# huttered40/capital

Measured on AMD Instinct MI355X. Metric: TFLOP/s (whole node) Cholesky n=65536, algorithmic n^3/3, recursive cholinv factor(), inputs resident in HBM, higher is better.
Workload: dtype f64

## Files before the change

capital_amd/csrc/capi_internal.h:

```cpp
#pragma once
#include <hip/hip_runtime.h>
#include <stdint.h>
#include <stdio.h>
#include <string.h>
#include "capital_hip.h"

struct capi_handle_s {
  int device = 0;
  hipStream_t stream = nullptr;
  bool owns_stream = false;
  static constexpr int NSTREAMS = 4;
  hipStream_t streams[NSTREAMS] = {nullptr, nullptr, nullptr, nullptr};
  int cur = 0;
  int cu_of[NSTREAMS] = {0, 0, 0, 0};
  hipEvent_t* events = nullptr;
  void* ws[NSTREAMS] = {nullptr, nullptr, nullptr, nullptr};
  size_t ws_bytes[NSTREAMS] = {0, 0, 0, 0};
  void* ws2[NSTREAMS] = {nullptr, nullptr, nullptr, nullptr};
  size_t ws2_bytes[NSTREAMS] = {0, 0, 0, 0};
  void* ws3[NSTREAMS] = {nullptr, nullptr, nullptr, nullptr};
  size_t ws3_bytes[NSTREAMS] = {0, 0, 0, 0};
  void* ws4[NSTREAMS] = {nullptr, nullptr, nullptr, nullptr};
  size_t ws4_bytes[NSTREAMS] = {0, 0, 0, 0};
  int* d_info = nullptr;
// ... 32 lines not shown
  do {                                                                                       \
    hipError_t e__ = (call);                                                                 \
    if (e__ != hipSuccess) {                                                                 \
      if (h) snprintf((h)->err, sizeof((h)->err), "%s:%d %s -> %s", __FILE__, __LINE__, #call, hipGetErrorString(e__)); \
      return CAPI_EHIP;                                                                      \
    }                                                                                        \
  } while (0)

#define CAPI_REQUIRE(h, cond, msg)                                                           \
  do {                                                                                       \
    if (!(cond)) {                                                                           \
      if (h) snprintf((h)->err, sizeof((h)->err), "%s:%d invalid argument: %s", __FILE__, __LINE__, msg); \
      return CAPI_EINVAL;                                                                    \
    }                                                                                        \
  } while (0)

int capi_ws_get(capi_handle_t h, size_t bytes, void** p);
int capi_ws2_get(capi_handle_t h, size_t bytes, void** p);
int capi_ws3_get(capi_handle_t h, size_t bytes, void** p);
int capi_ws4_get(capi_handle_t h, size_t bytes, void** p);

static inline int64_t cdiv(int64_t a, int64_t b) { return (a + b - 1) / b; }

hipError_t capi_release(capi_handle_t h, void* p);
```

capital_amd/csrc/gemm_f64.hip:

```cpp
#include "capi_internal.h"
#include "gemm_plan.h"
#include <type_traits>

extern "C" int capi_internal_copy2d(capi_handle_t h, int64_t m, int64_t n, const double* A, int64_t lda, double* B, int64_t ldb);

typedef double d4_t __attribute__((ext_vector_type(4)));
typedef double d2_t __attribute__((ext_vector_type(2)));

namespace {

constexpr int NTHREADS = 256;
using gemm_plan::BK, gemm_plan::SK;
template <int TS> struct tile_cfg {
  static constexpr int TILE_LDS = TS * SK;
  static constexpr int STAGE_LDS = 2 * TILE_LDS;
  static constexpr int NQ = TS / 32;
  static constexpr int SUB = TS / 32;
};
constexpr int GROUP_M = 8;
template <int TS> __device__ __forceinline__ int rc_r(int tid, int q) { return 16 * ((tid >> 6) * (TS / 64) + (q >> 1)) + 2 * (tid & 7); }
__device__ __forceinline__ int rc_k(int tid, int q) { return 8 * (q & 1) + ((tid >> 3) & 7); }

struct GemmArgs {
  const double* A;
  const double* B;
  double* C;
  int64_t lda, ldb, ldc;
  int M, N, K;
  double alpha, beta;
  int out_uplo;
  int tri_side;
  int tri_eff_upper;
  int tri_unit;
  int a_vec, b_vec;
  int splitk, k_per_split;
  int k_rotate;
  double* slab;
  int64_t slab_ld, slab_stride;
  int tiles_m, tiles_n, ntiles;
  int batch;
  int64_t sa, sb, sc;
  int tail_base, tail_tm, tail_tn;
  int ts;
  int no_skip;
  int share_ab;
  int tri_dense;
  int tri_koff;
  int tri_block;
  int pid_base;
  int order;
// ... 396 lines not shown
  } else if (p.beta == 0.0) {
#pragma unroll
    for (int a = 0; a < SUB; ++a) {
      const int i = i0 + wm * (TS / 2) + a * 16 + r16;
#pragma unroll
      for (int b = 0; b < SUB; ++b)
#pragma unroll
        for (int reg = 0; reg < 4; ++reg) {
          const int j = j0 + wn * (TS / 2) + b * 16 + g + 4 * reg;
          if (element_ok(i, j)) p.C[i + (int64_t)j * p.ldc] = p.alpha * acc[a][b][reg];
        }
    }
  } else {
#pragma unroll
    for (int a = 0; a < SUB; ++a) {
      const int i = i0 + wm * (TS / 2) + a * 16 + r16;
      double old[SUB][4];
#pragma unroll
      for (int b = 0; b < SUB; ++b)
#pragma unroll
        for (int reg = 0; reg < 4; ++reg) {
          const int j = j0 + wn * (TS / 2) + b * 16 + g + 4 * reg;
          const bool ok = element_ok(i, j);
          old[b][reg] = *(ok ? p.C + i + (int64_t)j * p.ldc : p.C);
        }
#pragma unroll
      for (int b = 0; b < SUB; ++b)
#pragma unroll
        for (int reg = 0; reg < 4; ++reg) {
          const int j = j0 + wn * (TS / 2) + b * 16 + g + 4 * reg;
          if (element_ok(i, j)) p.C[i + (int64_t)j * p.ldc] = p.alpha * acc[a][b][reg] + p.beta * old[b][reg];
        }
    }
  }
  stamp_end(p);
}

template <bool AK, bool BKC>
__global__ __launch_bounds__(NTHREADS, 2) void dtrmm_pair_kernel(const GemmArgs p) {
  constexpr int TS = 128, BM = TS, BN = TS, SUB = tile_cfg<TS>::SUB, NQ = tile_cfg<TS>::NQ;
  constexpr int NW = NQ * ((AK ? 1 : 2) + (BKC ? 1 : 2));
  constexpr int TILE_LDS = tile_cfg<TS>::TILE_LDS, STAGE_LDS = tile_cfg<TS>::STAGE_LDS;
  constexpr int kstep = BK;
  extern __shared__ __attribute__((aligned(16))) double lds[];
  const int tid = threadIdx.x;
  const int lane = tid & 63, wave = tid >> 6;
  const int r16 = lane & 15, g = lane >> 4;
// ... 146 lines not shown
        const int tn = t + dir;
        iterate(t, (tn >= 0 && tn < ntk) ? tn : -1, std::false_type{});
        t = tn;
        if (t >= 0 && t < ntk && fast_run(t) > 0) break;
      }
    }

#pragma unroll
    for (int a = 0; a < SUB; ++a) {
      const int i = i0 + wm * (TS / 2) + a * 16 + r16;
#pragma unroll
      for (int c = 0; c < SUB; ++c)
#pragma unroll
        for (int reg = 0; reg < 4; ++reg) {
          const int j = j0 + wn * (TS / 2) + c * 16 + g + 4 * reg;
          p.C[i + (int64_t)j * p.ldc] = p.alpha * acc[a][c][reg];
        }
    }
  }
  stamp_end(p);
}

__global__ void splitk_reduce_kernel(const double* __restrict__ slab, int64_t slab_ld, int64_t slab_stride, int splitk,
                                     double* __restrict__ C, int64_t ldc, int M, int N, double alpha, double beta, int out_uplo) {
  const int i = blockIdx.x * blockDim.x + threadIdx.x;
  if (i >= M) return;
  for (int j = blockIdx.y; j < N; j += gridDim.y) {
    if (out_uplo == CAPI_UPPER && i > j) continue;
    if (out_uplo == CAPI_LOWER && i < j) continue;
    double s = 0.0;
    for (int z = 0; z < splitk; ++z) s += slab[(int64_t)z * slab_stride + i + (int64_t)j * slab_ld];
    double* c = C + i + (int64_t)j * ldc;
    double r = alpha * s;
    if (beta != 0.0) r += beta * (*c);
    *c = r;
  }
}

__global__ __launch_bounds__(256) void splitk_reduce_wide_kernel(const double* __restrict__ slab, int64_t slab_ld, int64_t slab_stride,
                                                                 int splitk, double* __restrict__ C, int64_t ldc, int M, int N,
                                                                 double alpha, double beta, int out_uplo) {
  __shared__ double part[4][64];
  const int il = threadIdx.x & 63, zl = threadIdx.x >> 6;
  const int i = blockIdx.x * 64 + il, j = blockIdx.y;
  const bool live = i < M && !(out_uplo == CAPI_UPPER && i > j) && !(out_uplo == CAPI_LOWER && i < j);
  double s = 0.0;
  if (live) {
    const double* src = slab + i + (int64_t)j * slab_ld;
    int z = zl;
    for (; z + 28 < splitk; z += 32) {
      double v[8];
#pragma unroll
      for (int q = 0; q < 8; ++q) v[q] = src[(int64_t)(z + 4 * q) * slab_stride];
#pragma unroll
      for (int q = 0; q < 8; ++q) s += v[q];
    }
    for (; z < splitk; z += 4) s += src[(int64_t)z * slab_stride];
  }
  part[zl][il] = s;
  __syncthreads();
  if (zl == 0 && live) {
    const double t = ((part[0][il] + part[1][il]) + part[2][il]) + part[3][il];
    double* c = C + i + (int64_t)j * ldc;
    double r = alpha * t;
    if (beta != 0.0) r += beta * (*c);
    *c = r;
  }
}

__global__ void scale_kernel(double* __restrict__ C, int64_t ldc, int M, int N, double beta, int out_uplo) {
  const int i = blockIdx.x * blockDim.x + threadIdx.x;
  if (i >= M) return;
  for (int j = blockIdx.y; j < N; j += gridDim.y) {
    if (out_uplo == CAPI_UPPER && i > j) continue;
    if (out_uplo == CAPI_LOWER && i < j) continue;
    double* c = C + i + (int64_t)j * ldc;
    *c = beta == 0.0 ? 0.0 : beta * (*c);
  }
}

typedef void (*gemm_kernel_t)(const GemmArgs);

using gemm_plan::ST, gemm_plan::SKC, gemm_plan::SQK, gemm_plan::SLD;

template <bool KC>
__device__ __forceinline__ void small_load(const double* __restrict__ X, int64_t ld, int r0, int R, int kc, int kend, int tid,
                                           bool vec_ok, int quarter, d2_t (&v)[16]) {
#pragma unroll
  for (int qq = 0; qq < 4; ++qq) {
    const int q = 4 * quarter + qq;
    int r[2], k[2];
    if (KC) { r[0] = r[1] = r0 + (tid >> 3); k[0] = kc + 2 * (tid & 7) + 16 * q; k[1] = k[0] + 1; }
    else { r[0] = r0 + 2 * (tid & 15); r[1] = r[0] + 1; k[0] = k[1] = kc + (tid >> 4) + 16 * q; }
    const double* ptr = KC ? X + (int64_t)r[0] * ld + k[0] : X + (int64_t)k[0] * ld + r[0];
    const bool in = r[1] < R && k[1] < kend && vec_ok;
    v[q] = *(const d2_t*)(in ? ptr : X);
  }
}

template <bool KC>
// ... 40 lines not shown

template <bool KC>
__device__ __forceinline__ void small_store(double* __restrict__ L, int tid, int quarter, const d2_t (&v)[16]) {
#pragma unroll
  for (int qq = 0; qq < 4; ++qq) {
    const int q = 4 * quarter + qq;
    if (KC) {
      const int k = 2 * (tid & 7) + 16 * q, r = tid >> 3;
      L[k * SLD + r] = v[q].x;
      L[(k + 1) * SLD + r] = v[q].y;
    } else {
      const int k = (tid >> 4) + 16 * q, r = 2 * (tid & 15);
      *(d2_t*)&L[k * SLD + r] = v[q];
    }
  }
}

template <bool AK, bool BKC>
__global__ __launch_bounds__(256, 1) void dgemm_small_kernel(const GemmArgs pin) {
  extern __shared__ __attribute__((aligned(16))) double lds[];
  GemmArgs p = pin;
  if (p.batch > 1) {
    const int64_t bz = blockIdx.y;
    p.A += bz * p.sa; p.B += bz * p.sb; p.C += bz * p.sc;
  }
  double* La = lds;
  double* Lb = lds + p.ts * SLD;
  const int tid = threadIdx.x, lane = tid & 63, wave = tid >> 6;
  const int r16 = lane & 15, g = lane >> 4, wm = wave & 1, wn = wave >> 1;
  const int ti = blockIdx.x % p.tiles_m, tj = blockIdx.x / p.tiles_m;
  const int i0 = ti * ST, j0 = tj * ST;
  if (p.out_uplo == CAPI_UPPER && i0 > j0 + ST - 1) return;
  if (p.out_uplo == CAPI_LOWER && j0 > i0 + ST - 1) return;
  int klo = 0, khi = p.K;
  if (p.tri_side == CAPI_LEFT) {
    if (p.tri_eff_upper) klo = i0; else khi = min(p.K, i0 + ST);
  } else if (p.tri_side == CAPI_RIGHT) {
    if (p.tri_eff_upper) khi = min(p.K, j0 + ST); else klo = j0;
  }
  klo &= ~1;
  const bool keep_ge = (p.tri_side == CAPI_LEFT) == (p.tri_eff_upper != 0);
  d4_t acc = {0.0, 0.0, 0.0, 0.0};
  for (int kc = klo; kc < khi; kc += SKC) {
    d2_t va[16], vb[16];
    const int span = khi - kc < SKC ? khi - kc : SKC;
    const bool fast = p.a_vec && p.b_vec && i0 + ST <= p.M && j0 + ST <= p.N && (span & 15) == 0;
    if (fast) {
// ... 20 lines not shown
      }
      small_store<AK>(La, tid, quarter, va);
      small_store<BKC>(Lb, tid, quarter, vb);
      __syncthreads();
#pragma unroll
      for (int s4 = 0; s4 < SQK / 4; ++s4) {
        const int k = quarter * SQK + 4 * s4 + g;
        const double a = La[k * SLD + wm * 16 + r16];
        const double b = Lb[k * SLD + wn * 16 + r16];
        acc = __builtin_amdgcn_mfma_f64_16x16x4f64(b, a, acc, 0, 0, 0);
      }
    }
  }
  const int i = i0 + wm * 16 + r16;
  double old[4];
  bool okv[4];
#pragma unroll
  for (int reg = 0; reg < 4; ++reg) {
    const int j = j0 + wn * 16 + g + 4 * reg;
    bool ok = (i < p.M) && (j < p.N);
    if (p.out_uplo == CAPI_UPPER) ok = ok && (i <= j);
    if (p.out_uplo == CAPI_LOWER) ok = ok && (i >= j);
    okv[reg] = ok;
    old[reg] = (p.beta != 0.0) ? *(ok ? p.C + i + (int64_t)j * p.ldc : p.C) : 0.0;
  }
#pragma unroll
  for (int reg = 0; reg < 4; ++reg) {
    const int j = j0 + wn * 16 + g + 4 * reg;
    if (okv[reg]) p.C[i + (int64_t)j * p.ldc] = p.alpha * acc[reg] + (p.beta != 0.0 ? p.beta * old[reg] : 0.0);
  }
}

gemm_kernel_t pick_small(bool ak, bool bkc) {
  return ak ? (bkc ? dgemm_small_kernel<true, true> : dgemm_small_kernel<true, false>)
            : (bkc ? dgemm_small_kernel<false, true> : dgemm_small_kernel<false, false>);
}



constexpr int TSK_THREADS = 512;
using gemm_plan::TSK_W;

template <int W, bool FULLW>
__device__ __forceinline__ void gram_ts_body(const GemmArgs& p, double* __restrict__ lds) {
  constexpr int STAGE = TSK_W * SK;
  constexpr int RA = W, RB = 15 - W, NA = 16 - RA;
  const int tid = threadIdx.x, lane = tid & 63;
// ... 85 lines not shown
  }
  __syncthreads();
  int it = 0;
  if (FULLW && p.a_vec && p.K % BK == 0) {
    for (; it + 3 < np; it += 2) {
      step(it, stB, stA, std::true_type{});
      step(it + 1, stA, stB, std::true_type{});
    }
  }
  for (; it < np; it += 2) {
    step(it, stB, stA, std::false_type{});
    if (it + 1 < np) step(it + 1, stA, stB, std::false_type{});
  }
  auto put = [&](int trow, int tcol, const d4_t& v) {
    const int i = 16 * trow + r16;
#pragma unroll
    for (int reg = 0; reg < 4; ++reg) {
      const int j = 16 * tcol + g + 4 * reg;
      if (i < N && j < N && i <= j) {
        if (p.splitk > 1) p.slab[(int64_t)z * p.slab_stride + i + (int64_t)j * p.slab_ld] = v[reg];
        else {
          double* c = p.C + i + (int64_t)j * p.ldc;
          double r = p.alpha * v[reg];
          if (p.beta != 0.0) r += p.beta * (*c);
          *c = r;
        }
      }
    }
  };
#pragma unroll
  for (int j = RA; j < 16; ++j) if (j < nct) put(RA, j, acc[j - RA]);
#pragma unroll
  for (int j = RB; j < 16; ++j) if (j < nct) put(RB, j, acc[NA + j - RB]);
}

__global__ __launch_bounds__(TSK_THREADS, 1) void gram_ts_kernel(const GemmArgs p) {
  extern __shared__ __attribute__((aligned(16))) double lds[];
  const int w = __builtin_amdgcn_readfirstlane(threadIdx.x >> 6);
  if (p.N == TSK_W) {
    switch (w) {
      case 0: gram_ts_body<0, true>(p, lds); break;
      case 1: gram_ts_body<1, true>(p, lds); break;
      case 2: gram_ts_body<2, true>(p, lds); break;
      case 3: gram_ts_body<3, true>(p, lds); break;
      case 4: gram_ts_body<4, true>(p, lds); break;
      case 5: gram_ts_body<5, true>(p, lds); break;
      case 6: gram_ts_body<6, true>(p, lds); break;
// ... 179 lines not shown
      h->prof_cap = ncap;
    }
    rec = &h->prof[h->prof_n++];
    if (!rec->e0) { CAPI_HIP_CHECK(h, hipEventCreate(&rec->e0)); CAPI_HIP_CHECK(h, hipEventCreate(&rec->e1)); }
    rec->flops = q.out_uplo >= 0 ? (double)q.N * ((double)q.N + 1.0) * (double)q.K
                 : (q.tri_side >= 0 ? (q.tri_block ? (double)q.M * (double)q.N * (2.0 * (double)q.tri_koff + (double)q.N) : (double)q.M * (double)q.N * (double)q.K)
                                    : 2.0 * (double)q.M * (double)q.N * (double)q.K);
    rec->flops *= share;
    rec->variant = variant;
    rec->m = q.M; rec->n = q.N; rec->k = q.K; rec->kind = q.out_uplo >= 0 ? 1 : (q.tri_side >= 0 ? 2 : 0);
    CAPI_HIP_CHECK(h, hipEventRecord(rec->e0, h->stream));
    const int64_t idx = rec - h->prof;
    q.stamp = h->d_stamps && idx < h->stamps_cap ? h->d_stamps + 2 * idx : nullptr;
  }
  hipLaunchKernelGGL(k, dim3((unsigned)grid), dim3(NTHREADS), lds_bytes, h->stream, q);
  if (rec) CAPI_HIP_CHECK(h, hipEventRecord(rec->e1, h->stream));
  return CAPI_OK;
}

int launch_reduce(capi_handle_t h, const GemmArgs& p, gemm_plan::Reduce kind) {
  if (kind == gemm_plan::Reduce::none) return CAPI_OK;
  if (kind == gemm_plan::Reduce::wide)
    hipLaunchKernelGGL(splitk_reduce_wide_kernel, dim3((unsigned)cdiv(p.M, 64), (unsigned)p.N), dim3(256), 0, h->stream, p.slab, p.slab_ld,
                       p.slab_stride, p.splitk, p.C, p.ldc, p.M, p.N, p.alpha, p.beta, p.out_uplo);
  else
    hipLaunchKernelGGL(splitk_reduce_kernel, dim3((unsigned)cdiv(p.M, 256), (unsigned)(p.N < 65535 ? p.N : 65535)), dim3(256), 0, h->stream,
                       p.slab, p.slab_ld, p.slab_stride, p.splitk, p.C, p.ldc, p.M, p.N, p.alpha, p.beta, p.out_uplo);
  CAPI_HIP_CHECK(h, hipGetLastError());
  return CAPI_OK;
}

int launch_gemm(capi_handle_t h, bool ak, bool bkc, GemmArgs& p, bool ws_for_slab) {
  using gemm_plan::Path;
  const GemmEnv& env = gemm_env();
  gemm_plan::Product d;
  d.M = p.M; d.N = p.N; d.K = p.K; d.out_uplo = p.out_uplo;
  d.tri_side = p.tri_side; d.tri_eff_upper = p.tri_eff_upper; d.tri_dense = p.tri_dense; d.tri_block = p.tri_block; d.tri_koff = p.tri_koff;
  d.alpha_zero = p.alpha == 0.0; d.beta = p.beta; d.batch = p.batch; d.ak = ak; d.bkc = bkc;
  d.a_is_b = p.A == p.B; d.same_ld = p.lda == p.ldb;
  d.a_vec = (((uintptr_t)p.A & 15) == 0) && ((p.lda & 1) == 0);
  d.b_vec = (((uintptr_t)p.B & 15) == 0) && ((p.ldb & 1) == 0);
  d.a_tiled = p.a_tiled; d.c_tiled = p.c_tiled; d.ws_for_slab = ws_for_slab;
  const gemm_plan::Device dev{h->num_cu, h->cu_of[h->cur]};
  const gemm_plan::Modes modes{h->rounds_mode, h->pair_mode, h->pair_rounds, h->pair_rounds_min};
  const gemm_plan::Plan pl = gemm_plan::plan(d, dev, modes, env.ov);
  if (env.debug) {
    char line[2048];
    gemm_plan::format(line, sizeof(line), d, dev, modes, env.ov, pl);
    fprintf(stderr, "[capi gemm] %s\n", line);
  }
  hipStream_t s = h->stream;
  if (pl.path == Path::none) return CAPI_OK;
  CAPI_REQUIRE(h, pl.path != Path::refused, "panel32 operand reached a kernel that does not read it");
  if (pl.path == Path::scale) {
    dim3 grid((unsigned)cdiv(p.M, 256), (unsigned)(p.N < 65535 ? p.N : 65535));
    hipLaunchKernelGGL(scale_kernel, grid, dim3(256), 0, s, p.C, p.ldc, p.M, p.N, p.beta, p.out_uplo);
    CAPI_HIP_CHECK(h, hipGetLastError());
    return CAPI_OK;
  }
  if (pl.path == Path::trmm_ts32) {
    p.a_vec = d.a_vec;
    p.splitk = 1;
    CAPI_RAISE_LDS_LIMIT(h, CAPI_ATTR_TRMM_TS32, trmm_right_ts32_kernel, pl.lds_bytes);
    hipLaunchKernelGGL(trmm_right_ts32_kernel, dim3((unsigned)pl.blocks), dim3(TSK_THREADS), pl.lds_bytes, s, p);
    CAPI_HIP_CHECK(h, hipGetLastError());
    return CAPI_OK;
  }
  if (pl.path == Path::gram_blocks) {
    for (int J = 0; J < pl.tiles_n; ++J)
      for (int I = 0; I <= J; ++I) {
        GemmArgs q = p;
        q.A = p.A + (int64_t)I * TSK_W * p.lda;
        q.B = p.A + (int64_t)J * TSK_W * p.lda;
        q.C = p.C + (int64_t)I * TSK_W + (int64_t)J * TSK_W * p.ldc;
        q.M = q.N = TSK_W;
        q.out_uplo = I == J ? CAPI_UPPER : -1;
        int rc = launch_gemm(h, true, true, q, true);
        if (rc != CAPI_OK) return rc;
      }
    return CAPI_OK;
  }
  if (pl.path == Path::gram_ts) {
    p.a_vec = d.a_vec;
    p.splitk = pl.splitk;
    p.slab = nullptr; p.slab_ld = pl.slab_ld; p.slab_stride = pl.slab_stride;
    if (pl.reduce != gemm_plan::Reduce::none) {
      void* ws;
      int rc = capi_ws_get(h, sizeof(double) * (size_t)p.slab_stride * (size_t)p.splitk, &ws);
      if (rc != CAPI_OK) return rc;
      p.slab = (double*)ws;
    }
    CAPI_RAISE_LDS_LIMIT(h, CAPI_ATTR_GRAM_TS, gram_ts_kernel, pl.lds_bytes);
    hipLaunchKernelGGL(gram_ts_kernel, dim3((unsigned)pl.blocks), dim3(TSK_THREADS), pl.lds_bytes, s, p);
    CAPI_HIP_CHECK(h, hipGetLastError());
    return launch_reduce(h, p, pl.reduce);
  }
  p.ts = pl.ts;
// ... 85 lines not shown
    CAPI_REQUIRE(h, A && B, "null operand");
    CAPI_REQUIRE(h, lda >= (transA ? k : m) && ldb >= (transB ? n : k), "lda/ldb");
  }
  GemmArgs p{};
  p.A = A; p.B = B; p.C = C; p.lda = lda; p.ldb = ldb; p.ldc = ldc;
  p.M = (int)m; p.N = (int)n; p.K = (int)k; p.alpha = alpha; p.beta = beta;
  p.out_uplo = -1; p.tri_side = -1;
  return launch_gemm(h, transA == CAPI_TRANS, transB == CAPI_NOTRANS, p, true);
}

int capi_dgemmt(capi_handle_t h, int uplo, int transA, int transB, int64_t n, int64_t k, double alpha,
                const double* A, int64_t lda, const double* B, int64_t ldb, double beta, double* C, int64_t ldc) {
  CAPI_REQUIRE(h, h, "null handle");
  CAPI_REQUIRE(h, ok01(uplo) && ok01(transA) && ok01(transB), "enum code");
  CAPI_REQUIRE(h, n >= 0 && k >= 0 && n < (1LL << 31) && k < (1LL << 31), "dims");
  if (n == 0) return CAPI_OK;
  CAPI_REQUIRE(h, C && ldc >= n, "C/ldc");
  if (k > 0) {
    CAPI_REQUIRE(h, A && B, "null operand");
    CAPI_REQUIRE(h, lda >= (transA ? k : n) && ldb >= (transB ? n : k), "lda/ldb");
  }
  GemmArgs p{};
  p.A = A; p.B = B; p.C = C; p.lda = lda; p.ldb = ldb; p.ldc = ldc;
  p.M = (int)n; p.N = (int)n; p.K = (int)k; p.alpha = alpha; p.beta = beta;
  p.out_uplo = uplo; p.tri_side = -1;
  return launch_gemm(h, transA == CAPI_TRANS, transB == CAPI_NOTRANS, p, true);
}

int capi_dsyrk(capi_handle_t h, int uplo, int trans, int64_t n, int64_t k, double alpha,
               const double* A, int64_t lda, double beta, double* C, int64_t ldc) {
  CAPI_REQUIRE(h, h, "null handle");
  CAPI_REQUIRE(h, ok01(trans), "transpose code");
  return capi_dgemmt(h, uplo, trans, trans == CAPI_TRANS ? CAPI_NOTRANS : CAPI_TRANS, n, k, alpha, A, lda, A, lda, beta, C, ldc);
}

static int trmm_launch(capi_handle_t h, int side, int uplo, int trans, int diag, int64_t m, int64_t n, double alpha,
                       const double* T, int64_t ldt, const double* B, int64_t ldb, double beta, double* C, int64_t ldc,
                       bool ws_free = true) {
  CAPI_REQUIRE(h, h, "null handle");
  CAPI_REQUIRE(h, ok01(side) && ok01(uplo) && ok01(trans) && ok01(diag), "enum code");
  CAPI_REQUIRE(h, m >= 0 && n >= 0 && m < (1LL << 31) && n < (1LL << 31), "dims");
  if (m == 0 || n == 0) return CAPI_OK;
  const int64_t nt = side == CAPI_LEFT ? m : n;
  CAPI_REQUIRE(h, T && B && C && ldt >= nt && ldb >= m && ldc >= m, "operands");
  CAPI_REQUIRE(h, (const double*)C != B, "out-of-place trmm: C aliases B");
  GemmArgs p{};
// ... 223 lines not shown
```

capital_amd/src/alg/cholesky/cholinv/cholinv.h:

```cpp
#ifndef CAPITAL_CHOLESKY_CHOLINV_H_
#define CAPITAL_CHOLESKY_CHOLINV_H_

#include "./../../alg.h"
#include "./../../matmult/summa/summa.h"
#include "./policy.h"

#pragma weak capi_dtrmm_thin
#pragma weak capi_dresid_ts

namespace cholesky {

template <class SerializePolicy = policy::cholinv::Serialize, class IntermediatesPolicy = policy::cholinv::SaveIntermediates,
          class BaseCasePolicy = policy::cholinv::NoReplication>
class cholinv : public SerializePolicy, public IntermediatesPolicy, public BaseCasePolicy {
public:
  using SP = SerializePolicy;
  using IP = IntermediatesPolicy;
  using BP = BaseCasePolicy;

  template <typename ScalarT, typename DimensionT>
  class info {
  public:
    using ScalarType = ScalarT;
    using DimensionType = DimensionT;
    using alg_type = cholinv<SerializePolicy, IntermediatesPolicy, BaseCasePolicy>;
    using SP = SerializePolicy;
    using IP = IntermediatesPolicy;
    using BP = BaseCasePolicy;
    info(const info& p) : complete_inv(p.complete_inv), split(p.split), bc_mult_dim(p.bc_mult_dim), dir(p.dir) {}
    info(info&& p) : complete_inv(p.complete_inv), split(p.split), bc_mult_dim(p.bc_mult_dim), dir(p.dir) {}
    info(DimensionType complete_inv, DimensionType split, DimensionType bc_mult_dim, char dir)
        : complete_inv(complete_inv), split(split), bc_mult_dim(bc_mult_dim), dir(dir) {}
    const DimensionType complete_inv, split, bc_mult_dim;
    const char dir;
    matrix<ScalarType, DimensionType, typename SerializePolicy::structure> R, Rinv;
    matrix<ScalarType, DimensionType, rect> Rfull, Rinvfull;
    matmult::arena work;
    DimensionType localDimension = 0, globalDimension = 0, trueLocalDimension = 0, trueGlobalDimension = 0, bcDimension = 0;
    int64_t num_base_cases = 0, num_levels = 0;
    bool solve_with_trsm = false;
    int potrf_info = 0;
    bool zeroed = false;
    const double* input = nullptr;
    DimensionType early_split = 0;
    DimensionType input_lead = 0;
    int la_depth = 0;
    bool factored = false, factored_trsm = false;
    DimensionType top_split = 0;
    matrix<ScalarType, DimensionType, rect> X, SolveW1, SolveW2, SolveRho, SolveD, SolveNorm2;
    std::vector<double> solve_residual_norms;
  };

  template <typename MatrixType, typename ArgType, typename CommType>
  static void factor(const MatrixType& A, ArgType& args, CommType&& CommInfo) {
    CRITTER_START(CI::factor);
    using U = typename ArgType::DimensionType;
    static_assert(std::is_same<typename MatrixType::StructureType, rect>::value, "cholinv::factor takes a rect-structured input block");
    if (!(args.split > 0) || args.dir != 'U') throw std::invalid_argument("cholinv: split > 0 and dir == 'U' required (cholinv.hpp:9)");
    if (CommInfo.d > 1 && CommInfo.d % CommInfo.c) throw std::invalid_argument("cholinv: c must divide d (or d == 1)");
    args.factored = false;
    args.factored_trsm = args.solve_with_trsm;
    args.top_split = 0;
    if (args.solve_with_trsm) { factor_trsm(A, args, CommInfo); args.factored = true; CRITTER_STOP(CI::factor); return; }
    const U localDimension = A.num_rows_local(), globalDimension = A.num_rows_global();
    CAPITAL_CHECK(capi_stream_select(capital::handle(), 0));
    CAPITAL_CHECK(capi_reset_info(capital::handle()));
    args.potrf_info = 0;
    args.R._register_(A.num_columns_global(), A.num_rows_global(), CommInfo.d, CommInfo.d);
// ... 8 lines not shown
    const U ld = localDimension;
    if (!args.zeroed) {
      capital::dev_zero(R, ld * ld);
      capital::dev_zero(Ri, ld * ld);
      args.zeroed = true;
    }
    U bcDimLocal = (U)(CommInfo.c * CommInfo.d);
    U bcMult = args.bc_mult_dim;
    if (bcMult < 0) { bcMult = -bcMult; for (U i = 0; i < bcMult; ++i) bcDimLocal *= 2; } else { for (U i = 0; i < bcMult; ++i) bcDimLocal /= 2; }
    bcDimLocal = std::max<U>(1, bcDimLocal);
    bcDimLocal = std::min<U>(localDimension, bcDimLocal);
    bcDimLocal = localDimension / bcDimLocal;
    args.localDimension = args.trueLocalDimension = localDimension;
    args.globalDimension = args.trueGlobalDimension = globalDimension;
    args.bcDimension = (U)CommInfo.d * bcDimLocal;
    args.num_base_cases = args.num_levels = 0;

    const U h1 = localDimension >> args.split;
    args.input = A.data();
    args.early_split = 0;
    const bool will_split = !(((localDimension * (U)CommInfo.d) <= args.bcDimension) || (h1 < args.split));
    args.input_lead = 0;
    args.top_split = will_split ? h1 : 0;
    if (will_split && h1 > 0 && h1 < ld) {
      capi_handle_t hh = capital::handle();
      U lead = h1;
      if (args.split == 1 && CommInfo.d == 1 && CommInfo.c == 1) while (lead >= 8192 && lead % 2 == 0 && (lead >> 1) * (U)CommInfo.d > args.bcDimension) lead >>= 1;
      CAPITAL_CHECK(capi_dlacpy(hh, 1, lead, lead, A.data(), ld, R, ld));
      CAPITAL_CHECK(capi_event_record(hh, EV_INPUT_HEAD));
      CAPITAL_CHECK(capi_stream_select(hh, 1));
      CAPITAL_CHECK(capi_event_wait(hh, EV_INPUT_HEAD));
      if (lead < h1) {
        CAPITAL_CHECK(capi_dlacpy(hh, 0, lead, h1 - lead, A.data() + (int64_t)lead * ld, ld, R + (int64_t)lead * ld, ld));
        CAPITAL_CHECK(capi_dlacpy(hh, 1, h1 - lead, h1 - lead, A.data() + lead + (int64_t)lead * ld, ld, R + lead + (int64_t)lead * ld, ld));
        CAPITAL_CHECK(capi_event_record(hh, EV_INPUT_MID));
        args.input_lead = lead;
      }
      CAPITAL_CHECK(capi_dlacpy(hh, 0, h1, ld - h1, A.data() + (int64_t)h1 * ld, ld, R + (int64_t)h1 * ld, ld));
      CAPITAL_CHECK(capi_dlacpy(hh, 1, ld - h1, ld - h1, A.data() + h1 + (int64_t)h1 * ld, ld, R + h1 + (int64_t)h1 * ld, ld));
      CAPITAL_CHECK(capi_event_record(hh, EV_INPUT_REST));
      CAPITAL_CHECK(capi_stream_select(hh, 0));
      args.early_split = h1;
    } else {
      CAPITAL_CHECK(capi_dlacpy(capital::handle(), 1, ld, ld, A.data(), ld, R, ld));
    }


    const bool single = (CommInfo.d == 1 && CommInfo.c == 1);
    capital::launch_rounds_scope rounds(true);
    const U h = localDimension - (localDimension >> args.split);
    const U agg = args.bcDimension;
    int64_t need = single ? (int64_t)h * h + (int64_t)h * h / 3 + 1024 : (int64_t)(CommInfo.d == 1 ? 8 : 12) * h * h + 4 * (int64_t)agg * agg + 4096;
    args.work.reserve(need);

    args.la_depth = 0;
    invoke(args, CommInfo, R, Ri, ld, (U)0, localDimension, globalDimension);

    if (packed) {
      const U e = args.early_split;
      if (e > 0) {
        pack_block(args, CAPI_UPPERTRI, R, (double*)args.R.data(), ld, e, ld, e, ld);
        pack_block(args, CAPI_UPPERTRI, Ri, (double*)args.Rinv.data(), ld, e, ld, e, ld);
        if (args.complete_inv) pack_block(args, CAPI_RECT, Ri, (double*)args.Rinv.data(), ld, e, ld, 0, e);
        CAPITAL_CHECK(capi_event_wait(capital::handle(), EV_EARLY_PACK));
      } else {
        serialize<uppertri, uppertri>::invoke(args.Rfull, args.R, 0, ld, 0, ld, 0, ld, 0, ld);
        serialize<uppertri, uppertri>::invoke(args.Rinvfull, args.Rinv, 0, ld, 0, ld, 0, ld, 0, ld);
      }
    }
    if (!IP::keep_arena) {
      capital::sync();
      args.work.release();
      if (packed) { args.Rfull._destroy_(); args.Rinvfull._destroy_(); args.zeroed = false; }
    }
    CRITTER_STOP(CI::factor);
// ... 227 lines not shown
  }

  template <typename ArgType, typename CommType>
  static matrix<typename ArgType::ScalarType, typename ArgType::DimensionType, rect> construct_R(ArgType& args, CommType&& CommInfo) {
    return construct(args.R, CommInfo);
  }
  template <typename ArgType, typename CommType>
  static matrix<typename ArgType::ScalarType, typename ArgType::DimensionType, rect> construct_Rinv(ArgType& args, CommType&& CommInfo) {
    if (args.solve_with_trsm) throw std::logic_error("cholinv: the TRSM mode forms no inverse (info::solve_with_trsm)");
    return construct(args.Rinv, CommInfo);
  }

private:
  static constexpr int EV_INPUT_HEAD = 1020, EV_INPUT_REST = 1021, EV_TOP_R12 = 1022, EV_EARLY_PACK = 1023, EV_INPUT_MID = 1019;
  static constexpr int EV_BC_POTRF = 1008, EV_BC_SCATTER = 1009;
  static constexpr int EV_LA_LEAD = 1010, EV_LA_REST = 1014, LA_STREAM0 = 2, LA_MAX_DEPTH = 2;
  static int64_t lookahead_min() {
    if (getenv("CAPITAL_NO_LOOKAHEAD")) return -1;
    const char* e = getenv("CAPITAL_LOOKAHEAD_MIN");
    if (e) return (int64_t)atoll(e);
    return getenv("CAPITAL_LOOKAHEAD") ? (int64_t)2048 : -1;
  }

  static int lookahead_depth() {
    const char* e = getenv("CAPITAL_LA_DEPTH");
    return e ? std::max(0, std::min(atoi(e), (int)LA_MAX_DEPTH)) : (int)LA_MAX_DEPTH;
  }

  template <typename ArgType>
  static void pack_block(ArgType&, int shape, const double* full, double* packed_dst, int64_t ld, int64_t x0, int64_t x1, int64_t y0,
                         int64_t y1) {
    CAPITAL_CHECK(capi_serialize_shape(capital::handle(), shape, CAPI_RECT, CAPI_UPPERTRI, full, ld, ld, packed_dst, ld, ld,
                                       x0, x1, y0, y1, x0, x1, y0, y1));
  }

  template <typename M, typename CommType>
  static matrix<typename M::ScalarType, typename M::DimensionType, rect> construct(M& src, CommType&& CommInfo) {
    const auto ld = src.num_rows_local();
    matrix<typename M::ScalarType, typename M::DimensionType, rect> ret(src.num_columns_global(), src.num_rows_global(), CommInfo.d, CommInfo.d);
    serialize<typename SP::structure, rect>::invoke(src, ret, 0, ld, 0, ld, 0, ld, 0, ld);
    return ret;
  }

  template <typename ArgType, typename CommType, typename U>
  static void invoke(ArgType& args, CommType&& t, double* R, double* Ri, U ld, U start, U localDim, U globalDim, int wait_ev = -1) {
    using matmult::view;
// ... 1 lines not shown
    const U split1 = localDim >> args.split;
    if (((localDim * (U)t.d) <= args.bcDimension) || (split1 < args.split)) {
      if (wait_ev >= 0) CAPITAL_CHECK(capi_event_wait(h, wait_ev));
      CRITTER_START(CI::factor_diag);
      base_case(args, t, R, Ri, ld, start, localDim);
      CRITTER_STOP(CI::factor_diag);
      return;
    }
    ++args.num_levels;
    const U split2 = localDim - split1;
    const bool single = (t.d == 1 && t.c == 1);
    matmult::arena& ws = args.work;
    view R11i{Ri + start + start * ld, ld, split1, split1};
    view A12{R + start + (start + split1) * ld, ld, split1, split2};
    view A22{R + (start + split1) + (start + split1) * ld, ld, split2, split2};
    view R22i{Ri + (start + split1) + (start + split1) * ld, ld, split2, split2};
    view I12{Ri + start + (start + split1) * ld, ld, split1, split2};

    invoke(args, t, R, Ri, ld, start, split1, globalDim >> 1);
    if (wait_ev >= 0) CAPITAL_CHECK(capi_event_wait(h, wait_ev));
    if (start == 0 && args.input_lead > 0 && split1 == args.input_lead) CAPITAL_CHECK(capi_event_wait(h, EV_INPUT_MID));

    const bool top = (localDim == args.localDimension) && args.early_split == split1;
    if (top) CAPITAL_CHECK(capi_event_wait(h, EV_INPUT_REST));
    CRITTER_START(CI::trsm);
    int child_wait = -1;
    bool copy_deferred = false;
    const int64_t mark = ws.top;
    {
      view W{ws.take((int64_t)split1 * split2), split1, split1, split2};
      if (single) {
        CAPITAL_CHECK(capi_dtrmm_oop(h, CAPI_LEFT, CAPI_UPPER, CAPI_TRANS, CAPI_NONUNIT, split1, split2, 1.0, R11i.p, ld, A12.p, ld, W.p, W.ld));
      } else {
        view Tx{ws.take((int64_t)split1 * split1), split1, split1, split1};
        const int64_t np = matmult::summa::tri_count(split1);
        if ((t.x == t.y && !t.multipath) || !matmult::summa::packed_comm()) {
          CAPITAL_CHECK(capi_dlacpy(h, 0, split1, split1, R11i.p, ld, Tx.p, Tx.ld));
          util::transpose_raw(Tx.p, Tx.count(), ws.take(Tx.count()), t, matmult::summa::relay_space(t, Tx.count(), ws));
        } else if (t.x == t.y) {
          CAPITAL_CHECK(capi_dlacpy(h, 0, split1, split1, R11i.p, ld, Tx.p, Tx.ld));
          util::transpose_raw(nullptr, np, nullptr, t, matmult::summa::relay_space(t, np, ws));
        } else {
          double* pk = ws.take(np);
          matmult::summa::pack_tri(R11i, CAPI_UPPER, pk);
          util::transpose_raw(pk, np, ws.take(np), t, matmult::summa::relay_space(t, np, ws));
          matmult::summa::unpack_tri(pk, CAPI_UPPER, Tx);
        }
        matmult::summa::trmm(t, CAPI_LEFT, CAPI_UPPER, CAPI_TRANS, CAPI_NONUNIT, 1.0, Tx, A12, W, ws);
      }
      const U lead = split2 >> args.split;
      const bool a22_splits = !(((split2 * (U)t.d) <= args.bcDimension) || (lead < args.split));
      const bool la = single && a22_splits && lead > 0 && lookahead_min() >= 0 && (int64_t)split2 >= lookahead_min() && args.la_depth < lookahead_depth();
      const bool pack_now = top && !std::is_same<typename SP::structure, rect>::value;
      const bool copy_later = la && pack_now && !getenv("CAPITAL_PACK_AT_ONCE");
      if (!copy_later) CAPITAL_CHECK(capi_dlacpy(h, 0, split1, split2, W.p, W.ld, A12.p, ld));
      copy_deferred = copy_later;
      CRITTER_STOP(CI::trsm);
      auto early_pack = [&](int after_ev) {
        CAPITAL_CHECK(capi_stream_select(h, 1));
        CAPITAL_CHECK(capi_event_wait(h, after_ev));
        if (copy_later) CAPITAL_CHECK(capi_dlacpy(h, 0, split1, split2, W.p, W.ld, A12.p, ld));
        pack_block(args, CAPI_UPPERTRI, R, (double*)args.R.data(), ld, (U)0, split1, (U)0, split1);
        pack_block(args, CAPI_RECT, R, (double*)args.R.data(), ld, split1, ld, (U)0, split1);
        pack_block(args, CAPI_UPPERTRI, Ri, (double*)args.Rinv.data(), ld, (U)0, split1, (U)0, split1);
        CAPITAL_CHECK(capi_event_record(h, EV_EARLY_PACK));
        CAPITAL_CHECK(capi_stream_select(h, 0));
      };
      bool packed_early = false;

      CRITTER_START(CI::tmu);
      if (la) {
        const int depth = args.la_depth;
        const U rest = split2 - lead;
        double* Wr = W.p + (int64_t)lead * W.ld;
        CAPITAL_CHECK(capi_dgemmt(h, CAPI_UPPER, CAPI_TRANS, CAPI_NOTRANS, lead, split1, -1.0, W.p, W.ld, W.p, W.ld, 1.0, A22.p, ld));
        CAPITAL_CHECK(capi_event_record(h, EV_LA_LEAD + depth));
        CAPITAL_CHECK(capi_stream_select(h, LA_STREAM0 + depth));
        CAPITAL_CHECK(capi_event_wait(h, EV_LA_LEAD + depth));
        CAPITAL_CHECK(capi_dgemm(h, CAPI_TRANS, CAPI_NOTRANS, lead, rest, split1, -1.0, W.p, W.ld, Wr, W.ld, 1.0, A22.p + (int64_t)lead * ld, ld));
        CAPITAL_CHECK(capi_dgemmt(h, CAPI_UPPER, CAPI_TRANS, CAPI_NOTRANS, rest, split1, -1.0, Wr, W.ld, Wr, W.ld, 1.0,
                                  A22.p + lead + (int64_t)lead * ld, ld));
        CAPITAL_CHECK(capi_event_record(h, EV_LA_REST + depth));
        CAPITAL_CHECK(capi_stream_select(h, 0));
        child_wait = EV_LA_REST + depth;
        ++args.la_depth;
        if (pack_now && !getenv("CAPITAL_PACK_AT_ONCE")) { early_pack(EV_LA_REST + depth); packed_early = true; }
      } else if (single) {
        CAPITAL_CHECK(capi_dgemmt(h, CAPI_UPPER, CAPI_TRANS, CAPI_NOTRANS, split2, split1, -1.0, W.p, W.ld, W.p, W.ld, 1.0, A22.p, ld));
      } else {
        view Wx{ws.take(W.count()), split1, split1, split2};
        capital::dev_copy(Wx.p, W.p, W.count());
        util::transpose_raw(Wx.p, Wx.count(), ws.take(Wx.count()), t, matmult::summa::relay_space(t, Wx.count(), ws));
        matmult::summa::syrk(t, CAPI_UPPER, CAPI_TRANS, -1.0, W, Wx, 1.0, A22, ws);
      }
      if (pack_now && !packed_early) {
        CAPITAL_CHECK(capi_event_record(h, EV_TOP_R12));
        early_pack(EV_TOP_R12);
      }
      if (child_wait < 0) ws.top = mark;
      CRITTER_STOP(CI::tmu);
    }

    invoke(args, t, R, Ri, ld, start + split1, split2, split2 * (U)t.d, child_wait);
    if (child_wait >= 0) { --args.la_depth; ws.top = mark; }

    CRITTER_START(CI::tmu);
    if (!(!args.complete_inv && (globalDim == args.trueGlobalDimension))) {
      if (copy_deferred) CAPITAL_CHECK(capi_event_wait(h, EV_EARLY_PACK));
      const int64_t mark = ws.top;
// ... 123 lines not shown
```

Baseline: 55.49.

## Read top-level A12/A22 directly from input instead of copying into R first

Adds an out-of-place-accumulate gemmt variant (separate Cin source for the beta term) and uses it at the top recursion level so the trailing A22 update reads the original input and writes into R, and the TRMM writes A12 directly into R from input. This removes the two initial dlacpy copies of the upper-right and trailing blocks, plus the W workspace and copy-back for A12, lowering HBM traffic and workspace size. It only applies when not distributed and lookahead is not active at the top, and it drops the overlap of those input copies on a side stream.

```diff
diff --git a/capital_amd/csrc/capi_internal.h b/capital_amd/csrc/capi_internal.h
--- a/capital_amd/csrc/capi_internal.h
+++ b/capital_amd/csrc/capi_internal.h
@@ -78,4 +78,7 @@
 
 static inline int64_t cdiv(int64_t a, int64_t b) { return (a + b - 1) / b; }
 
+extern "C" int capi_dgemmt_acc(capi_handle_t h, int uplo, int transA, int transB, int64_t n, int64_t k, double alpha, const double* A, int64_t lda,
+                               const double* B, int64_t ldb, double beta, const double* Cin, int64_t ldcin, double* C, int64_t ldc);
+
 hipError_t capi_release(capi_handle_t h, void* p);
diff --git a/capital_amd/csrc/gemm_f64.hip b/capital_amd/csrc/gemm_f64.hip
--- a/capital_amd/csrc/gemm_f64.hip
+++ b/capital_amd/csrc/gemm_f64.hip
@@ -25,7 +25,8 @@
   const double* A;
   const double* B;
   double* C;
-  int64_t lda, ldb, ldc;
+  const double* Cin;
+  int64_t lda, ldb, ldc, ldcin;
   int M, N, K;
   double alpha, beta;
   int out_uplo;
@@ -468,7 +469,7 @@
         for (int reg = 0; reg < 4; ++reg) {
           const int j = j0 + wn * (TS / 2) + b * 16 + g + 4 * reg;
           const bool ok = element_ok(i, j);
-          old[b][reg] = *(ok ? p.C + i + (int64_t)j * p.ldc : p.C);
+          old[b][reg] = *(ok ? p.Cin + i + (int64_t)j * p.ldcin : p.Cin);
         }
 #pragma unroll
       for (int b = 0; b < SUB; ++b)
@@ -661,7 +662,8 @@
 }
 
 __global__ void splitk_reduce_kernel(const double* __restrict__ slab, int64_t slab_ld, int64_t slab_stride, int splitk,
-                                     double* __restrict__ C, int64_t ldc, int M, int N, double alpha, double beta, int out_uplo) {
+                                     double* C, int64_t ldc, const double* Cin, int64_t ldcin, int M, int N, double alpha, double beta,
+                                     int out_uplo) {
   const int i = blockIdx.x * blockDim.x + threadIdx.x;
   if (i >= M) return;
   for (int j = blockIdx.y; j < N; j += gridDim.y) {
@@ -671,14 +673,14 @@
     for (int z = 0; z < splitk; ++z) s += slab[(int64_t)z * slab_stride + i + (int64_t)j * slab_ld];
     double* c = C + i + (int64_t)j * ldc;
     double r = alpha * s;
-    if (beta != 0.0) r += beta * (*c);
+    if (beta != 0.0) r += beta * Cin[i + (int64_t)j * ldcin];
     *c = r;
   }
 }
 
 __global__ __launch_bounds__(256) void splitk_reduce_wide_kernel(const double* __restrict__ slab, int64_t slab_ld, int64_t slab_stride,
-                                                                 int splitk, double* __restrict__ C, int64_t ldc, int M, int N,
-                                                                 double alpha, double beta, int out_uplo) {
+                                                                 int splitk, double* C, int64_t ldc, const double* Cin,
+                                                                 int64_t ldcin, int M, int N, double alpha, double beta, int out_uplo) {
   __shared__ double part[4][64];
   const int il = threadIdx.x & 63, zl = threadIdx.x >> 6;
   const int i = blockIdx.x * 64 + il, j = blockIdx.y;
@@ -702,19 +704,18 @@
     const double t = ((part[0][il] + part[1][il]) + part[2][il]) + part[3][il];
     double* c = C + i + (int64_t)j * ldc;
     double r = alpha * t;
-    if (beta != 0.0) r += beta * (*c);
+    if (beta != 0.0) r += beta * Cin[i + (int64_t)j * ldcin];
     *c = r;
   }
 }
 
-__global__ void scale_kernel(double* __restrict__ C, int64_t ldc, int M, int N, double beta, int out_uplo) {
+__global__ void scale_kernel(double* C, int64_t ldc, const double* Cin, int64_t ldcin, int M, int N, double beta, int out_uplo) {
   const int i = blockIdx.x * blockDim.x + threadIdx.x;
   if (i >= M) return;
   for (int j = blockIdx.y; j < N; j += gridDim.y) {
     if (out_uplo == CAPI_UPPER && i > j) continue;
     if (out_uplo == CAPI_LOWER && i < j) continue;
-    double* c = C + i + (int64_t)j * ldc;
-    *c = beta == 0.0 ? 0.0 : beta * (*c);
+    C[i + (int64_t)j * ldc] = beta == 0.0 ? 0.0 : beta * Cin[i + (int64_t)j * ldcin];
   }
 }
 
@@ -801,7 +802,7 @@
   GemmArgs p = pin;
   if (p.batch > 1) {
     const int64_t bz = blockIdx.y;
-    p.A += bz * p.sa; p.B += bz * p.sb; p.C += bz * p.sc;
+    p.A += bz * p.sa; p.B += bz * p.sb; p.C += bz * p.sc; p.Cin += bz * p.sc;
   }
   double* La = lds;
   double* Lb = lds + p.ts * SLD;
@@ -868,7 +869,7 @@
     if (p.out_uplo == CAPI_UPPER) ok = ok && (i <= j);
     if (p.out_uplo == CAPI_LOWER) ok = ok && (i >= j);
     okv[reg] = ok;
-    old[reg] = (p.beta != 0.0) ? *(ok ? p.C + i + (int64_t)j * p.ldc : p.C) : 0.0;
+    old[reg] = (p.beta != 0.0) ? *(ok ? p.Cin + i + (int64_t)j * p.ldcin : p.Cin) : 0.0;
   }
 #pragma unroll
   for (int reg = 0; reg < 4; ++reg) {
@@ -1000,7 +1001,7 @@
         else {
           double* c = p.C + i + (int64_t)j * p.ldc;
           double r = p.alpha * v[reg];
-          if (p.beta != 0.0) r += p.beta * (*c);
+          if (p.beta != 0.0) r += p.beta * p.Cin[i + (int64_t)j * p.ldcin];
           *c = r;
         }
       }
@@ -1226,10 +1227,10 @@
   if (kind == gemm_plan::Reduce::none) return CAPI_OK;
   if (kind == gemm_plan::Reduce::wide)
     hipLaunchKernelGGL(splitk_reduce_wide_kernel, dim3((unsigned)cdiv(p.M, 64), (unsigned)p.N), dim3(256), 0, h->stream, p.slab, p.slab_ld,
-                       p.slab_stride, p.splitk, p.C, p.ldc, p.M, p.N, p.alpha, p.beta, p.out_uplo);
+                       p.slab_stride, p.splitk, p.C, p.ldc, p.Cin, p.ldcin, p.M, p.N, p.alpha, p.beta, p.out_uplo);
   else
     hipLaunchKernelGGL(splitk_reduce_kernel, dim3((unsigned)cdiv(p.M, 256), (unsigned)(p.N < 65535 ? p.N : 65535)), dim3(256), 0, h->stream,
-                       p.slab, p.slab_ld, p.slab_stride, p.splitk, p.C, p.ldc, p.M, p.N, p.alpha, p.beta, p.out_uplo);
+                       p.slab, p.slab_ld, p.slab_stride, p.splitk, p.C, p.ldc, p.Cin, p.ldcin, p.M, p.N, p.alpha, p.beta, p.out_uplo);
   CAPI_HIP_CHECK(h, hipGetLastError());
   return CAPI_OK;
 }
@@ -1237,6 +1238,7 @@
 int launch_gemm(capi_handle_t h, bool ak, bool bkc, GemmArgs& p, bool ws_for_slab) {
   using gemm_plan::Path;
   const GemmEnv& env = gemm_env();
+  if (!p.Cin) { p.Cin = p.C; p.ldcin = p.ldc; }
   gemm_plan::Product d;
   d.M = p.M; d.N = p.N; d.K = p.K; d.out_uplo = p.out_uplo;
   d.tri_side = p.tri_side; d.tri_eff_upper = p.tri_eff_upper; d.tri_dense = p.tri_dense; d.tri_block = p.tri_block; d.tri_koff = p.tri_koff;
@@ -1258,7 +1260,7 @@
   CAPI_REQUIRE(h, pl.path != Path::refused, "panel32 operand reached a kernel that does not read it");
   if (pl.path == Path::scale) {
     dim3 grid((unsigned)cdiv(p.M, 256), (unsigned)(p.N < 65535 ? p.N : 65535));
-    hipLaunchKernelGGL(scale_kernel, grid, dim3(256), 0, s, p.C, p.ldc, p.M, p.N, p.beta, p.out_uplo);
+    hipLaunchKernelGGL(scale_kernel, grid, dim3(256), 0, s, p.C, p.ldc, p.Cin, p.ldcin, p.M, p.N, p.beta, p.out_uplo);
     CAPI_HIP_CHECK(h, hipGetLastError());
     return CAPI_OK;
   }
@@ -1277,6 +1279,7 @@
         q.A = p.A + (int64_t)I * TSK_W * p.lda;
         q.B = p.A + (int64_t)J * TSK_W * p.lda;
         q.C = p.C + (int64_t)I * TSK_W + (int64_t)J * TSK_W * p.ldc;
+        q.Cin = p.Cin + (int64_t)I * TSK_W + (int64_t)J * TSK_W * p.ldcin;
         q.M = q.N = TSK_W;
         q.out_uplo = I == J ? CAPI_UPPER : -1;
         int rc = launch_gemm(h, true, true, q, true);
@@ -1408,6 +1411,25 @@
   }
   GemmArgs p{};
   p.A = A; p.B = B; p.C = C; p.lda = lda; p.ldb = ldb; p.ldc = ldc;
+  p.M = (int)n; p.N = (int)n; p.K = (int)k; p.alpha = alpha; p.beta = beta;
+  p.out_uplo = uplo; p.tri_side = -1;
+  return launch_gemm(h, transA == CAPI_TRANS, transB == CAPI_NOTRANS, p, true);
+}
+
+int capi_dgemmt_acc(capi_handle_t h, int uplo, int transA, int transB, int64_t n, int64_t k, double alpha, const double* A, int64_t lda,
+                    const double* B, int64_t ldb, double beta, const double* Cin, int64_t ldcin, double* C, int64_t ldc) {
+  CAPI_REQUIRE(h, h, "null handle");
+  CAPI_REQUIRE(h, ok01(uplo) && ok01(transA) && ok01(transB), "enum code");
+  CAPI_REQUIRE(h, n >= 0 && k >= 0 && n < (1LL << 31) && k < (1LL << 31), "dims");
+  if (n == 0) return CAPI_OK;
+  CAPI_REQUIRE(h, C && ldc >= n && Cin && ldcin >= n, "C/ldc, Cin/ldcin");
+  if (k > 0) {
+    CAPI_REQUIRE(h, A && B, "null operand");
+    CAPI_REQUIRE(h, lda >= (transA ? k : n) && ldb >= (transB ? n : k), "lda/ldb");
+  }
+  GemmArgs p{};
+  p.A = A; p.B = B; p.C = C; p.lda = lda; p.ldb = ldb; p.ldc = ldc;
+  p.Cin = Cin; p.ldcin = ldcin;
   p.M = (int)n; p.N = (int)n; p.K = (int)k; p.alpha = alpha; p.beta = beta;
   p.out_uplo = uplo; p.tri_side = -1;
   return launch_gemm(h, transA == CAPI_TRANS, transB == CAPI_NOTRANS, p, true);
diff --git a/capital_amd/src/alg/cholesky/cholinv/cholinv.h b/capital_amd/src/alg/cholesky/cholinv/cholinv.h
--- a/capital_amd/src/alg/cholesky/cholinv/cholinv.h
+++ b/capital_amd/src/alg/cholesky/cholinv/cholinv.h
@@ -7,6 +7,9 @@
 
 #pragma weak capi_dtrmm_thin
 #pragma weak capi_dresid_ts
+extern "C" int capi_dgemmt_acc(capi_handle_t h, int uplo, int transA, int transB, int64_t n, int64_t k, double alpha, const double* A, int64_t lda,
+                               const double* B, int64_t ldb, double beta, const double* Cin, int64_t ldcin, double* C, int64_t ldc);
+#pragma weak capi_dgemmt_acc
 
 namespace cholesky {
 
@@ -44,6 +47,7 @@
     const double* input = nullptr;
     DimensionType early_split = 0;
     DimensionType input_lead = 0;
+    bool top_from_input = false;
     int la_depth = 0;
     bool factored = false, factored_trsm = false;
     DimensionType top_split = 0;
@@ -98,6 +102,8 @@
     const bool will_split = !(((localDimension * (U)CommInfo.d) <= args.bcDimension) || (h1 < args.split));
     args.input_lead = 0;
     args.top_split = will_split ? h1 : 0;
+    args.top_from_input = will_split && h1 > 0 && h1 < ld && CommInfo.d == 1 && CommInfo.c == 1 && &capi_dgemmt_acc &&
+                          !lookahead_at(args, CommInfo, ld - h1, 0);
     if (will_split && h1 > 0 && h1 < ld) {
       capi_handle_t hh = capital::handle();
       U lead = h1;
@@ -112,9 +118,11 @@
         CAPITAL_CHECK(capi_event_record(hh, EV_INPUT_MID));
         args.input_lead = lead;
       }
-      CAPITAL_CHECK(capi_dlacpy(hh, 0, h1, ld - h1, A.data() + (int64_t)h1 * ld, ld, R + (int64_t)h1 * ld, ld));
-      CAPITAL_CHECK(capi_dlacpy(hh, 1, ld - h1, ld - h1, A.data() + h1 + (int64_t)h1 * ld, ld, R + h1 + (int64_t)h1 * ld, ld));
-      CAPITAL_CHECK(capi_event_record(hh, EV_INPUT_REST));
+      if (!args.top_from_input) {
+        CAPITAL_CHECK(capi_dlacpy(hh, 0, h1, ld - h1, A.data() + (int64_t)h1 * ld, ld, R + (int64_t)h1 * ld, ld));
+        CAPITAL_CHECK(capi_dlacpy(hh, 1, ld - h1, ld - h1, A.data() + h1 + (int64_t)h1 * ld, ld, R + h1 + (int64_t)h1 * ld, ld));
+        CAPITAL_CHECK(capi_event_record(hh, EV_INPUT_REST));
+      }
       CAPITAL_CHECK(capi_stream_select(hh, 0));
       args.early_split = h1;
     } else {
@@ -127,6 +135,7 @@
     const U h = localDimension - (localDimension >> args.split);
     const U agg = args.bcDimension;
     int64_t need = single ? (int64_t)h * h + (int64_t)h * h / 3 + 1024 : (int64_t)(CommInfo.d == 1 ? 8 : 12) * h * h + 4 * (int64_t)agg * agg + 4096;
+    if (args.top_from_input) need = (args.complete_inv ? (int64_t)h * h : ((int64_t)h * h + 3) / 4 + 2) + 1024;
     args.work.reserve(need);
 
     args.la_depth = 0;
@@ -400,6 +409,13 @@
     return getenv("CAPITAL_LOOKAHEAD") ? (int64_t)2048 : -1;
   }
 
+  template <typename ArgType, typename CommType, typename U>
+  static bool lookahead_at(ArgType& args, CommType&& t, U split2, int depth) {
+    const U lead = split2 >> args.split;
+    const bool a22_splits = !(((split2 * (U)t.d) <= args.bcDimension) || (lead < args.split));
+    return t.d == 1 && t.c == 1 && a22_splits && lead > 0 && lookahead_min() >= 0 && (int64_t)split2 >= lookahead_min() && depth < lookahead_depth();
+  }
+
   static int lookahead_depth() {
     const char* e = getenv("CAPITAL_LA_DEPTH");
     return e ? std::max(0, std::min(atoi(e), (int)LA_MAX_DEPTH)) : (int)LA_MAX_DEPTH;
@@ -447,14 +463,18 @@
     if (start == 0 && args.input_lead > 0 && split1 == args.input_lead) CAPITAL_CHECK(capi_event_wait(h, EV_INPUT_MID));
 
     const bool top = (localDim == args.localDimension) && args.early_split == split1;
-    if (top) CAPITAL_CHECK(capi_event_wait(h, EV_INPUT_REST));
+    const bool from_input = top && args.top_from_input;
+    if (top && !from_input) CAPITAL_CHECK(capi_event_wait(h, EV_INPUT_REST));
     CRITTER_START(CI::trsm);
     int child_wait = -1;
     bool copy_deferred = false;
     const int64_t mark = ws.top;
     {
-      view W{ws.take((int64_t)split1 * split2), split1, split1, split2};
-      if (single) {
+      view W = from_input ? A12 : view{ws.take((int64_t)split1 * split2), split1, split1, split2};
+      if (from_input) {
+        const double* A12in = args.input + (int64_t)split1 * ld;
+        CAPITAL_CHECK(capi_dtrmm_oop(h, CAPI_LEFT, CAPI_UPPER, CAPI_TRANS, CAPI_NONUNIT, split1, split2, 1.0, R11i.p, ld, A12in, ld, A12.p, ld));
+      } else if (single) {
         CAPITAL_CHECK(capi_dtrmm_oop(h, CAPI_LEFT, CAPI_UPPER, CAPI_TRANS, CAPI_NONUNIT, split1, split2, 1.0, R11i.p, ld, A12.p, ld, W.p, W.ld));
       } else {
         view Tx{ws.take((int64_t)split1 * split1), split1, split1, split1};
@@ -474,11 +494,10 @@
         matmult::summa::trmm(t, CAPI_LEFT, CAPI_UPPER, CAPI_TRANS, CAPI_NONUNIT, 1.0, Tx, A12, W, ws);
       }
       const U lead = split2 >> args.split;
-      const bool a22_splits = !(((split2 * (U)t.d) <= args.bcDimension) || (lead < args.split));
-      const bool la = single && a22_splits && lead > 0 && lookahead_min() >= 0 && (int64_t)split2 >= lookahead_min() && args.la_depth < lookahead_depth();
+      const bool la = lookahead_at(args, t, split2, args.la_depth);
       const bool pack_now = top && !std::is_same<typename SP::structure, rect>::value;
       const bool copy_later = la && pack_now && !getenv("CAPITAL_PACK_AT_ONCE");
-      if (!copy_later) CAPITAL_CHECK(capi_dlacpy(h, 0, split1, split2, W.p, W.ld, A12.p, ld));
+      if (!copy_later && !from_input) CAPITAL_CHECK(capi_dlacpy(h, 0, split1, split2, W.p, W.ld, A12.p, ld));
       copy_deferred = copy_later;
       CRITTER_STOP(CI::trsm);
       auto early_pack = [&](int after_ev) {
@@ -510,6 +529,9 @@
         child_wait = EV_LA_REST + depth;
         ++args.la_depth;
         if (pack_now && !getenv("CAPITAL_PACK_AT_ONCE")) { early_pack(EV_LA_REST + depth); packed_early = true; }
+      } else if (from_input) {
+        CAPITAL_CHECK(capi_dgemmt_acc(h, CAPI_UPPER, CAPI_TRANS, CAPI_NOTRANS, split2, split1, -1.0, W.p, W.ld, W.p, W.ld, 1.0,
+                                      args.input + split1 + (int64_t)split1 * ld, ld, A22.p, ld));
       } else if (single) {
         CAPITAL_CHECK(capi_dgemmt(h, CAPI_UPPER, CAPI_TRANS, CAPI_NOTRANS, split2, split1, -1.0, W.p, W.ld, W.p, W.ld, 1.0, A22.p, ld));
       } else {
```

New measurement: 55.47, median of 2. Within noise of the previous version (-0.0%).
